# MECLabTUDA/Lifelong-nnUNet

Measured on AMD Instinct MI355X. Metric: 3D patches/sec (whole node) + mean Dice vs ref, 5-level 3D Generic_UNet training step, higher is better.
Workload: dtype f16 (fp32 accumulate, fp32 master weights); 1 GPU; BASELINE configs[1]: nnUNetTrainerSequential.run_iteration, 160x192x160 patches, batch 2/GPU, num_pool 5, base 32, 3 logits; global_batch=2, parallelism=dp1, distinct_resident_batches=2, deterministic_wgrad=False

## Files before the change

lifelong-nnunet_amd/csrc/igemm_conv.hip:

```cpp
#include "lnn_common.h"
#include "igemm_common.h"
#include "igemm_gen.h"
#include <cstdlib>

namespace {

typedef unsigned c1_uint4 __attribute__((ext_vector_type(4)));

template <bool STATS>
__global__ __launch_bounds__(256, 3) void conv_c1_fwd_kernel(const ConvParams p, int tiles_per_sample) {
    constexpr int TZ = 4, TY = 8, TX = 8, VT = TZ * TY * TX / 128, PZ = TZ + 2, PY = TY + 2, PX = TX + 2, P = PZ * PY * PX;
    constexpr int NL = (P + 255) / 256;
    __shared__ half_t xl[P];
    __shared__ float sred[STATS ? 4 * 2 * 32 : 1];
    const int tid = threadIdx.x, lane = tid & 63, wave = tid >> 6;
    const int n = blockIdx.y;
    const int m0 = blockIdx.z * 32;
    const long xbase_n = (long)n * p.Di * p.Hi * p.Wi;
    const int v = lane & 31, hk = lane >> 5;
    half8 a[2];
#pragma unroll
    for (int k16 = 0; k16 < 2; ++k16) a[k16] = *reinterpret_cast<const half8*>(p.wp + lnn_panel_off(0, m0 + v, k16 * 16 + hk * 8, 1, 32));
    int toff[2][8];
#pragma unroll
// ... 158 lines not shown
extern "C" int lnn_debug_set_gen_mode(int mode) {
    LNN_REQUIRE(mode >= -1 && mode <= 1, "lnn_debug_set_gen_mode: %d is not one of -1, 0, 1", mode);
    g_gen_mode = mode;
    return LNN_OK;
}
bool lnn_gen_prefers(int op, long voxels) {
    if (g_gen_mode >= 0) return g_gen_mode == 1;
    if (g_force_conv >= 0) return false;
    static int off = -1;
    if (off < 0) { const char* e = getenv("LNN_GEN"); off = (e && e[0] == '0') ? 1 : 0; }
    if (off) return false;
    switch (op) {
        case LNN_GEN_OP_CONV_S1: return voxels > 512 && voxels <= 4096;
        case LNN_GEN_OP_CONV_S2: return voxels <= 4096;
        case LNN_GEN_OP_CONVT_DGRAD: return voxels <= 20000;
        default: return false;
    }
}

namespace {
int check_act(const void* ptr, int ld, int C, const char* what) {
    LNN_REQUIRE(ptr != nullptr, "%s: null pointer", what);
    LNN_REQUIRE(lnn_aligned16(ptr), "%s: pointer not 16-byte aligned", what);
    LNN_REQUIRE(C > 0 && C % 8 == 0, "%s: channel count %d must be a positive multiple of 8", what, C);
    LNN_REQUIRE(ld >= C && ld % 8 == 0, "%s: ld %d must be >= C (%d) and a multiple of 8", what, ld, C);
    return LNN_OK;
}

}

// ... 328 lines not shown
```

lifelong-nnunet_amd/csrc/igemm_gen.h:

```cpp
#pragma once
#include "lnn_common.h"

typedef unsigned GenTap;
static inline GenTap gen_tap(int dz, int dy, int dx, int slot) {
    return (unsigned)(dz + 8) | ((unsigned)(dy + 8) << 8) | ((unsigned)(dx + 8) << 16) | ((unsigned)slot << 24);
}

struct GenParams {
    const half_t* x = nullptr;
    const half_t* wp = nullptr;
    const float* bias = nullptr;
    half_t* y = nullptr;
    float* scratch = nullptr;
    int ld_x = 0, ld_y = 0;
    int N = 0, Di = 0, Hi = 0, Wi = 0, Do = 0, Ho = 0, Wo = 0, Ld = 0, Lh = 0, Lw = 0;
    int soz = 1, soy = 1, sox = 1, siz = 1, siy = 1, six = 1;
    int C = 0, M = 0, Mpad = 0, KCpad = 0, wtaps = 0;
    int nclass = 0;
    int accumulate = 0, ksplit = 1;
    int vgroups = 0, mgroups = 0, nbpc = 0, xcd_order = 0;
    unsigned x_bytes = 0, wp_bytes = 0;
    GenTap taps[27] = {};
    unsigned cls_first[9] = {};
    unsigned cls_par[8] = {};
};

struct GenWParams {
    const half_t* p = nullptr;
    const half_t* q = nullptr;
    float* dwp = nullptr;
    float* parts = nullptr;
    long parts_elems = 0, part_stride = 0;
    int ld_p = 0, ld_q = 0;
    int N = 0, Ld = 0, Lh = 0, Lw = 0, Qd = 0, Qh = 0, Qw = 0;
    int siz = 1, siy = 1, six = 1;
    int M = 0, C = 0, Mpad = 0, Cpad = 0;
    int ntaps = 0, wtaps = 0, tgroups = 0, vparts = 1;
    unsigned p_bytes = 0, q_bytes = 0;
    GenTap taps[27] = {};
};

int lnn_gen_geometry(GenParams& p, int kind, const int k[3], const int st[3]);
int lnn_launch_gen(hipStream_t s, GenParams& p, float* ws, long ws_elems, const char* name);
int lnn_launch_gen_wgrad(hipStream_t s, GenWParams& p, const char* name);

int lnn_gen_conv3d_fwd(hipStream_t s, const void* x, int ld_x, const void* wp, const float* bias, void* y, int ld_y, int N, int Di,
                       int Hi, int Wi, int C, int K, const int k[3], const int st[3], float* ws, long ws_elems);
int lnn_gen_conv3d_dgrad(hipStream_t s, const void* dy, int ld_dy, const void* wp, void* dx, int ld_dx, int N, int Di, int Hi, int Wi,
                         int C, int K, const int k[3], const int st[3], int accumulate, float* ws, long ws_elems);
int lnn_gen_convT3d_fwd(hipStream_t s, const void* x, int ld_x, const void* wp, void* y, int ld_y, int N, int D, int H, int W, int C,
                        int K, const int st[3], float* ws, long ws_elems);
int lnn_gen_convT3d_dgrad(hipStream_t s, const void* dy, int ld_dy, const void* wp, void* dx, int ld_dx, int N, int D, int H, int W,
                          int C, int K, const int st[3], int accumulate, float* ws, long ws_elems);
int lnn_gen_conv3d_wgrad(hipStream_t s, const void* x, int ld_x, const void* dy, int ld_dy, float* dwp, int N, int Di, int Hi, int Wi,
                         int C, int K, const int k[3], const int st[3], float* parts, long parts_elems);
int lnn_gen_convT3d_wgrad(hipStream_t s, const void* x, int ld_x, const void* dy, int ld_dy, float* dwp, int N, int D, int H, int W,
                          int C, int K, const int st[3], float* parts, long parts_elems);
enum { LNN_GEN_OP_CONV_S1 = 0, LNN_GEN_OP_CONV_S2 = 1, LNN_GEN_OP_CONVT_FWD = 2, LNN_GEN_OP_CONVT_DGRAD = 3, LNN_GEN_OP_WGRAD = 4 };
bool lnn_gen_prefers(int op, long voxels);
```

lifelong-nnunet_amd/csrc/igemm_gen.hip:

```cpp
#include "igemm_common.h"
#include "igemm_gen.h"
#include <algorithm>

namespace {

typedef unsigned uint4v __attribute__((ext_vector_type(4)));
constexpr unsigned OOB = 0x80000000u;

__device__ __forceinline__ __amdgpu_buffer_rsrc_t gen_rsrc(const void* base, unsigned bytes) {
    return __builtin_amdgcn_make_buffer_rsrc(const_cast<void*>(base), 0, (int)bytes, 0x00020000);
}
__device__ __forceinline__ half8 gen_load16(__amdgpu_buffer_rsrc_t rs, unsigned off) {
    const uint4v r = __builtin_amdgcn_raw_buffer_load_b128(rs, (int)off, 0, 0);
    return __builtin_bit_cast(half8, r);
}

template <int RB, int VB, int D>
__global__ __launch_bounds__(256) void igemm_gen_kernel(const GenParams p) {
    const int lane = threadIdx.x & 63, wave = __builtin_amdgcn_readfirstlane(threadIdx.x >> 6);
    const int v = lane & 31, hk = lane >> 5;
    const int W = p.nclass * p.mgroups * p.ksplit;
    int w, vq;
    if (p.xcd_order) {
        const int xcd = blockIdx.x & 7, j = blockIdx.x >> 3;
// ... 121 lines not shown
                if (p.accumulate) {
                    const half4 old = *dst;
                    r0 += (float)old[0]; r1 += (float)old[1]; r2 += (float)old[2]; r3 += (float)old[3];
                }
                const half4 o = {(half_t)r0, (half_t)r1, (half_t)r2, (half_t)r3};
                *dst = o;
            }
        }
    }
}

typedef __attribute__((address_space(3))) void lds_void;
__device__ __forceinline__ void gen_dma16(__amdgpu_buffer_rsrc_t rs, char* lds_wave_base, unsigned voffset) {
    __builtin_amdgcn_raw_ptr_buffer_load_lds(rs, (lds_void*)lds_wave_base, 16, (int)voffset, 0, 0, 0);
}
__device__ __forceinline__ half4 gen_tr16(const char* addr) {
    fp16x4_t r = __builtin_amdgcn_ds_read_tr16_b64_v4f16((__attribute__((address_space(3))) fp16x4_t*)(addr));
    half4 o;
    __builtin_memcpy(&o, &r, 8);
    return o;
}
__device__ __forceinline__ half8 gen_tr_operand(const char* img, int p_addr) {
    const half4 lo = gen_tr16(img + p_addr), hi = gen_tr16(img + 256 + p_addr);
    half8 o;
#pragma unroll
    for (int i = 0; i < 4; ++i) { o[i] = lo[i]; o[4 + i] = hi[i]; }
    return o;
}
__device__ __forceinline__ int gen_div(int q, int d, float rd) {
    int r = (int)((float)q * rd);
    int rem = q - r * d;
    if (rem < 0) { --r; rem += d; }
    if (rem >= d) ++r;
    return r;
}

constexpr int GW_IMG = 1024;

template <int TPW>
__global__ __launch_bounds__(256) void igemm_gen_wgrad_kernel(const GenWParams p) {
    constexpr int WAVE_LDS = 2 * (1 + TPW) * GW_IMG;
    extern __shared__ __attribute__((aligned(16))) char smem[];
    const int lane = threadIdx.x & 63, wave = __builtin_amdgcn_readfirstlane(threadIdx.x >> 6);
    char* const lds = smem + wave * WAVE_LDS;
    const int panels = (p.Mpad >> 5) * (p.Cpad >> 5);
    const long units = (long)panels * p.tgroups * p.vparts;
    const long unit = (long)blockIdx.x * 4 + wave;
    if (unit >= units) return;
    const int vpart = (int)(unit % p.vparts);
    const int tg = (int)((unit / p.vparts) % p.tgroups);
    const int panel = (int)(unit / ((long)p.vparts * p.tgroups));
    const int m0 = (panel / (p.Cpad >> 5)) * 32, c0 = (panel % (p.Cpad >> 5)) * 32;
    const int t_begin = tg * TPW;
    const __amdgpu_buffer_rsrc_t rs_q = gen_rsrc(p.q, p.q_bytes);
    const __amdgpu_buffer_rsrc_t rs_p = gen_rsrc(p.p, p.p_bytes);

    const int dv = lane >> 2, dc = (lane & 3) * 8;
    const unsigned pcol = (m0 + dc < p.M) ? (unsigned)(m0 + dc) * 2u : OOB;
    const unsigned qcol = (c0 + dc < p.C) ? (unsigned)(c0 + dc) * 2u : OOB;
    const int hk = lane >> 5, cb = 16 * ((lane >> 4) & 1), sj = (lane & 15) >> 2, sq = lane & 3;
    const int p_addr = (8 * hk + sj) * 64 + (cb + 4 * sq) * 2;
    int tdz[TPW], tdy[TPW], tdx[TPW];
    unsigned tdead[TPW];
#pragma unroll
    for (int k = 0; k < TPW; ++k) {
        const bool has = t_begin + k < p.ntaps;
        const GenTap t = p.taps[has ? t_begin + k : 0];
        tdz[k] = (int)(t & 255) - 8; tdy[k] = (int)((t >> 8) & 255) - 8; tdx[k] = (int)((t >> 16) & 255) - 8;
        tdead[k] = has ? 0u : OOB;
    }

    floatx16 acc[TPW];
#pragma unroll
    for (int i = 0; i < TPW; ++i)
#pragma unroll
        for (int k = 0; k < 16; ++k) acc[i][k] = 0.f;

    const int total = p.N * p.Ld * p.Lh * p.Lw;
    const int groups = (total + 15) >> 4;
    const int g_begin = (int)((long)vpart * groups / p.vparts), g_end = (int)((long)(vpart + 1) * groups / p.vparts);
    const float rLw = 1.0f / (float)p.Lw, rLh = 1.0f / (float)p.Lh, rLd = 1.0f / (float)p.Ld;
    const unsigned prowb = (unsigned)p.ld_p * 2u, qrowb = (unsigned)p.ld_q * 2u;
#pragma unroll 1
    for (int gi = g_begin; gi < g_end; ++gi) {
        char* const buf = lds + (gi & 1) * (1 + TPW) * GW_IMG;
        const int q = gi * 16 + dv;
        const unsigned vdead = q < total ? 0u : OOB;
        const int qq = q < total ? q : 0;
        const int t1 = gen_div(qq, p.Lw, rLw), lx = qq - t1 * p.Lw;
        const int t2 = gen_div(t1, p.Lh, rLh), ly = t1 - t2 * p.Lh;
        const int n = gen_div(t2, p.Ld, rLd), lz = t2 - n * p.Ld;
        gen_dma16(rs_p, buf, (((unsigned)qq * prowb) | vdead | (pcol & OOB)) + (pcol & ~OOB));
        const int bz = lz * p.siz, by = ly * p.siy, bx = lx * p.six;
#pragma unroll
        for (int k = 0; k < TPW; ++k) {
            const int iz = bz + tdz[k], iy = by + tdy[k], ix = bx + tdx[k];
            const bool in = (unsigned)iz < (unsigned)p.Qd && (unsigned)iy < (unsigned)p.Qh && (unsigned)ix < (unsigned)p.Qw;
            const unsigned qrow = ((((unsigned)n * p.Qd + iz) * p.Qh + iy) * p.Qw + ix) * qrowb;
            gen_dma16(rs_q, buf + (1 + k) * GW_IMG, ((in ? qrow : OOB) | vdead | tdead[k] | (qcol & OOB)) + (qcol & ~OOB));
        }
        __builtin_amdgcn_s_waitcnt(0x0f70);
        __asm__ volatile("" ::: "memory");
        const half8 a = gen_tr_operand(buf, p_addr);
#pragma unroll
        for (int k = 0; k < TPW; ++k) {
            const half8 b = gen_tr_operand(buf + (1 + k) * GW_IMG, p_addr);
            acc[k] = __builtin_amdgcn_mfma_f32_32x32x16_f16(a, b, acc[k], 0, 0, 0);
        }
    }
    const int c = c0 + (lane & 31);
#pragma unroll
    for (int k = 0; k < TPW; ++k) {
        if (t_begin + k >= p.ntaps) continue;
        const int slot = (int)(p.taps[t_begin + k] >> 24);
#pragma unroll
        for (int i = 0; i < 16; ++i) {
            const int m = m0 + (i >> 2) * 8 + hk * 4 + (i & 3);
            const long idx = ((long)slot * p.Mpad + m) * p.Cpad + c;
            if (p.parts) p.parts[(long)vpart * p.part_stride + idx] = acc[k][i];
            else atomicAdd(p.dwp + idx, acc[k][i]);
        }
    }
}
// ... 90 lines not shown
    p.xcd_order = W % 8 == 0 ? 1 : 0;
    const unsigned grid = (unsigned)((long)W * p.nbpc);
    hipLaunchKernelGGL((igemm_gen_kernel<RB, VB, D>), dim3(grid), dim3(256), 0, s, p);
    LNN_CHECK_LAUNCH(name);
    if (ks > 1) {
        ConvParams c{};
        c.scratch = ws; c.ksplit = ks; c.Mpad = p.Mpad; c.M = p.M; c.bias = p.bias; c.y = p.y;
        c.ld_y = p.ld_y; c.accumulate = p.accumulate; c.N = p.N; c.Do = p.Do; c.Ho = p.Ho; c.Wo = p.Wo;
        return lnn_launch_splitk_finalize(s, c, name);
    }
    return LNN_OK;
}

template <int TPW>
static int gen_wgrad_launch_t(hipStream_t s, GenWParams& p, const char* name) {
    constexpr int WAVE_LDS = 2 * (1 + TPW) * GW_IMG;
    const long total = (long)p.N * p.Ld * p.Lh * p.Lw;
    p.tgroups = lnn_cdiv(p.ntaps, TPW);
    const long base = (long)(p.Mpad >> 5) * (p.Cpad >> 5) * p.tgroups;
    const int groups = (int)((total + 15) / 16);
    long vp = lnn_cdiv(8L * gen_num_cu(), base);
    if (vp > groups) vp = groups;
    if (vp < 1) vp = 1;
    const long slot_elems = (long)p.wtaps * p.Mpad * p.Cpad;
    if (p.parts) {
        while (vp > 1 && vp * slot_elems > p.parts_elems) --vp;
        LNN_REQUIRE(vp * slot_elems <= p.parts_elems, "%s: deterministic scratch too small (%ld floats needed, %ld given)", name,
                    vp * slot_elems, p.parts_elems);
        p.part_stride = slot_elems;
    }
    p.vparts = (int)vp;
    const long units = base * vp;
    auto kern = igemm_gen_wgrad_kernel<TPW>;
    static bool attr_set = false;
    if (!attr_set) {
        (void)hipFuncSetAttribute(reinterpret_cast<const void*>(kern), hipFuncAttributeMaxDynamicSharedMemorySize, 160 * 1024);
        attr_set = true;
    }
    hipLaunchKernelGGL(kern, dim3((unsigned)lnn_cdiv(units, 4)), dim3(256), (size_t)4 * WAVE_LDS, s, p);
    LNN_CHECK_LAUNCH(name);
    if (p.parts) {
        const long v4 = slot_elems / 4;
        const int blocks = (int)((v4 + 255) / 256 < 2048 ? (v4 + 255) / 256 : 2048);
        hipLaunchKernelGGL(gen_reduce_parts_kernel, dim3(blocks), dim3(256), 0, s, p.parts, (int)vp, slot_elems, p.dwp);
        LNN_CHECK_LAUNCH(name);
    }
    return LNN_OK;
}

int lnn_launch_gen_wgrad(hipStream_t s, GenWParams& p, const char* name) {
    const long total = (long)p.N * p.Ld * p.Lh * p.Lw;
    LNN_REQUIRE(total < (1L << 24), "%s: %ld loop voxels exceed the 2^24 the generic weight gradient indexes", name, total);
    const long pb = total * p.ld_p * 2, qb = (long)p.N * p.Qd * p.Qh * p.Qw * p.ld_q * 2;
    LNN_REQUIRE(pb < 0x7fffffffL && qb < 0x7fffffffL, "%s: tensor exceeds the 2 GB a buffer descriptor of the generic kernel covers", name);
    p.p_bytes = (unsigned)pb; p.q_bytes = (unsigned)qb;
    p.Mpad = lnn_round_up(p.M, 32); p.Cpad = lnn_round_up(p.C, 32);
    switch (p.ntaps) {
        case 27: return gen_wgrad_launch_t<7>(s, p, name);
        case 9: case 3: return gen_wgrad_launch_t<3>(s, p, name);
        case 8: case 4: return gen_wgrad_launch_t<4>(s, p, name);
        case 2: return gen_wgrad_launch_t<2>(s, p, name);
        case 1: return gen_wgrad_launch_t<1>(s, p, name);
    }
    lnn_set_error("%s: %d taps unsupported", name, p.ntaps);
    return LNN_ERR_BAD_ARG;
}

namespace {
int gen_check_act(const void* ptr, int ld, int C, const char* what) {
    LNN_REQUIRE(ptr != nullptr, "%s: null pointer", what);
    LNN_REQUIRE(lnn_aligned16(ptr), "%s: pointer not 16-byte aligned", what);
    LNN_REQUIRE(C > 0 && C % 8 == 0, "%s: channel count %d must be a positive multiple of 8", what, C);
    LNN_REQUIRE(ld >= C && ld % 8 == 0, "%s: ld %d must be >= C (%d) and a multiple of 8", what, ld, C);
    return LNN_OK;
// ... 64 lines not shown

int lnn_gen_convT3d_dgrad(hipStream_t s, const void* dy, int ld_dy, const void* wp, void* dx, int ld_dx, int N, int D, int H, int W,
                          int C, int K, const int st[3], int accumulate, float* ws, long ws_elems) {
    if (int e = gen_check_geom(st, st, true, "lnn_convT3d_dgrad_g")) return e;
    if (int e = gen_check_act(dy, ld_dy, K, "lnn_convT3d_dgrad_g(dy)")) return e;
    if (int e = gen_check_act(dx, ld_dx, C, "lnn_convT3d_dgrad_g(dx)")) return e;
    LNN_REQUIRE(wp != nullptr && lnn_aligned16(wp), "lnn_convT3d_dgrad_g: weight panel null/misaligned");
    GenParams p{};
    p.x = (const half_t*)dy; p.wp = (const half_t*)wp; p.y = (half_t*)dx; p.ld_x = ld_dy; p.ld_y = ld_dx;
    p.N = N; p.Di = D * st[0]; p.Hi = H * st[1]; p.Wi = W * st[2]; p.Do = D; p.Ho = H; p.Wo = W;
    p.Ld = D; p.Lh = H; p.Lw = W; p.C = K; p.M = C; p.accumulate = accumulate;
    lnn_gen_geometry(p, 3, st, st);
    return lnn_launch_gen(s, p, ws, ws_elems, "lnn_convT3d_dgrad_g");
}

int lnn_gen_conv3d_wgrad(hipStream_t s, const void* x, int ld_x, const void* dy, int ld_dy, float* dwp, int N, int Di, int Hi, int Wi,
                         int C, int K, const int k[3], const int st[3], float* parts, long parts_elems) {
    if (int e = gen_check_geom(k, st, false, "lnn_conv3d_wgrad_g")) return e;
    if (int e = gen_check_act(x, ld_x, C, "lnn_conv3d_wgrad_g(x)")) return e;
    if (int e = gen_check_act(dy, ld_dy, K, "lnn_conv3d_wgrad_g(dy)")) return e;
    LNN_REQUIRE(dwp != nullptr, "lnn_conv3d_wgrad_g: null panel");
    GenWParams p{};
    p.p = (const half_t*)dy; p.q = (const half_t*)x; p.dwp = dwp; p.ld_p = ld_dy; p.ld_q = ld_x; p.parts = parts; p.parts_elems = parts_elems;
    p.N = N; p.Qd = Di; p.Qh = Hi; p.Qw = Wi;
    p.Ld = (Di - 1) / st[0] + 1; p.Lh = (Hi - 1) / st[1] + 1; p.Lw = (Wi - 1) / st[2] + 1;
    p.siz = st[0]; p.siy = st[1]; p.six = st[2]; p.M = K; p.C = C;
    GenParams g{};
    p.ntaps = lnn_gen_geometry(g, 0, k, st);
    p.wtaps = g.wtaps;
    for (int t = 0; t < p.ntaps; ++t) p.taps[t] = g.taps[t];
    return lnn_launch_gen_wgrad(s, p, "lnn_conv3d_wgrad_g");
}

int lnn_gen_convT3d_wgrad(hipStream_t s, const void* x, int ld_x, const void* dy, int ld_dy, float* dwp, int N, int D, int H, int W,
                          int C, int K, const int st[3], float* parts, long parts_elems) {
    if (int e = gen_check_geom(st, st, true, "lnn_convT3d_wgrad_g")) return e;
    if (int e = gen_check_act(x, ld_x, C, "lnn_convT3d_wgrad_g(x)")) return e;
// ... 14 lines not shown
                                int Di, int Hi, int Wi, int C, int K, int kz, int ky, int kx, int sz, int sy, int sx, float* splitk_ws,
                                long splitk_elems) {
    const int k[3] = {kz, ky, kx}, st[3] = {sz, sy, sx};
    return lnn_gen_conv3d_fwd((hipStream_t)s, x, ld_x, wp, bias, y, ld_y, N, Di, Hi, Wi, C, K, k, st, splitk_ws, splitk_elems);
}
extern "C" int lnn_conv3d_dgrad_g(lnn_stream_t s, const void* dy, int ld_dy, const void* wp, void* dx, int ld_dx, int N, int Di, int Hi,
                                  int Wi, int C, int K, int kz, int ky, int kx, int sz, int sy, int sx, int accumulate, float* splitk_ws,
                                  long splitk_elems) {
    const int k[3] = {kz, ky, kx}, st[3] = {sz, sy, sx};
    return lnn_gen_conv3d_dgrad((hipStream_t)s, dy, ld_dy, wp, dx, ld_dx, N, Di, Hi, Wi, C, K, k, st, accumulate, splitk_ws, splitk_elems);
}
extern "C" int lnn_conv3d_wgrad_g(lnn_stream_t s, const void* x, int ld_x, const void* dy, int ld_dy, float* dwp, int N, int Di, int Hi,
                                  int Wi, int C, int K, int kz, int ky, int kx, int sz, int sy, int sx, float* parts, long parts_elems) {
    const int k[3] = {kz, ky, kx}, st[3] = {sz, sy, sx};
    LNN_REQUIRE(parts == nullptr || lnn_aligned16(parts), "lnn_conv3d_wgrad_g: scratch misaligned");
    return lnn_gen_conv3d_wgrad((hipStream_t)s, x, ld_x, dy, ld_dy, dwp, N, Di, Hi, Wi, C, K, k, st, parts, parts_elems);
}
extern "C" int lnn_convT3d_fwd_g(lnn_stream_t s, const void* x, int ld_x, const void* wp, void* y, int ld_y, int N, int D, int H, int W,
                                 int C, int K, int sz, int sy, int sx, float* splitk_ws, long splitk_elems) {
    const int st[3] = {sz, sy, sx};
    return lnn_gen_convT3d_fwd((hipStream_t)s, x, ld_x, wp, y, ld_y, N, D, H, W, C, K, st, splitk_ws, splitk_elems);
}
extern "C" int lnn_convT3d_dgrad_g(lnn_stream_t s, const void* dy, int ld_dy, const void* wp, void* dx, int ld_dx, int N, int D, int H,
                                   int W, int C, int K, int sz, int sy, int sx, int accumulate, float* splitk_ws, long splitk_elems) {
    const int st[3] = {sz, sy, sx};
    return lnn_gen_convT3d_dgrad((hipStream_t)s, dy, ld_dy, wp, dx, ld_dx, N, D, H, W, C, K, st, accumulate, splitk_ws, splitk_elems);
}
extern "C" int lnn_convT3d_wgrad_g(lnn_stream_t s, const void* x, int ld_x, const void* dy, int ld_dy, float* dwp, int N, int D, int H,
                                   int W, int C, int K, int sz, int sy, int sx, float* parts, long parts_elems) {
    const int st[3] = {sz, sy, sx};
    LNN_REQUIRE(parts == nullptr || lnn_aligned16(parts), "lnn_convT3d_wgrad_g: scratch misaligned");
// ... 3 lines not shown
```

lifelong-nnunet_amd/csrc/igemm_wgrad.hip:

```cpp
#include "lnn_common.h"
#include "igemm_gen.h"
#include <cstdlib>

namespace {

struct WTapTable {
    int ntaps;
    unsigned short pos_off[27];
    unsigned char slot[27];
};

struct WgradParams {
    const half_t* p;
    const half_t* q;
    const half_t* q2 = nullptr;
    int csplit = 0x7fffffff;
    float* dwp;
    int ld_p, ld_q;
    int N, Ld, Lh, Lw, Qd, Qh, Qw;
    int M, C, Mpad, Cpad;
    int tiles_z, tiles_y, tiles_x, tiles_total, tiles_per_block;
    int pad_lo;
    float* parts = nullptr;
    long parts_elems = 0, part_stride = 0;
// ... 955 lines not shown
        p.Cpad = 32;
        p.tiles_z = lnn_cdiv(p.Ld, TZ); p.tiles_y = lnn_cdiv(p.Lh, TY); p.tiles_x = lnn_cdiv(p.Lw, 8);
        p.tiles_total = N * p.tiles_z * p.tiles_y * p.tiles_x;
        int tpb = lnn_cdiv(p.tiles_total, 2048);
        if (tpb < 1) tpb = 1;
        p.tiles_per_block = tpb;
        dim3 grid((unsigned)lnn_cdiv(p.tiles_total, tpb), (unsigned)(p.Mpad / 32));
        const long slot_elems = (long)p.Mpad * 32;
        if (int e = wg_prepare_parts(p, grid.x, 4, slot_elems, "lnn_conv3d_wgrad(C=1)")) return e;
        if (p.gz) hipLaunchKernelGGL((wgrad_c1_kernel<TZ, TY, true>), grid, dim3(256), 0, s, p);
        else hipLaunchKernelGGL((wgrad_c1_kernel<TZ, TY, false>), grid, dim3(256), 0, s, p);
        LNN_CHECK_LAUNCH("lnn_conv3d_wgrad(C=1)");
        return wg_reduce_parts(s, p, grid.x, slot_elems, "lnn_conv3d_wgrad(C=1,reduce)");
    }
    if (int e = check_act_w(x, ld_x, x2 ? c_a : C, "lnn_conv3d_wgrad(x)")) return e;
    if (!x2 && lnn_gen_prefers(LNN_GEN_OP_WGRAD, (long)N * p.Ld * p.Lh * p.Lw)) {
        const int k3[3] = {3, 3, 3}, st3[3] = {stride, stride, stride};
        return lnn_gen_conv3d_wgrad(s, x, ld_x, dy, ld_dy, dwp, N, Di, Hi, Wi, C, K, k3, st3, parts, parts_elems);
    }
    p.taps.ntaps = 27;
    if (stride == 1) {
        constexpr int PY = 10, PX = 10;
        for (int t = 0; t < 27; ++t) {
            p.taps.pos_off[t] = (unsigned short)(((t / 9) * PY + (t / 3) % 3) * PX + t % 3);
            p.taps.slot[t] = (unsigned char)t;
        }
        LNN_REQUIRE(6L * p.Qh * p.Qw * p.ld_q * 2 < 0x7fffffffL && 4L * p.Lh * p.Lw * p.ld_p * 2 < 0x7fffffffL,
                    "lnn_conv3d_wgrad: a z-plane of %ld bytes is beyond the 2 GB window of the tile descriptors", (long)p.Qh * p.Qw * p.ld_q * 2);
        return launch_wgrad_s1_v5(s, p);
    }
    return launch_wgrad_s2<3>(s, p, "lnn_conv3d_wgrad(s2)");
}
}
// ... 70 lines not shown
```

lifelong-nnunet_amd/csrc/norm_act.hip:

```cpp
#include "igemm_common.h"

namespace {

constexpr int NT = 256;
typedef float float2v __attribute__((ext_vector_type(2)));
constexpr int MAX_BLOCKS = 1024;
constexpr int UNR = 4;

__device__ __forceinline__ half8 ld8(const half_t* p, int nt) {
    return nt ? __builtin_nontemporal_load(reinterpret_cast<const half8*>(p)) : *reinterpret_cast<const half8*>(p);
}
__device__ __forceinline__ void st8(half_t* p, const half8& v, int nt) {
    if (nt) __builtin_nontemporal_store(v, reinterpret_cast<half8*>(p));
    else *reinterpret_cast<half8*>(p) = v;
}
int in_nt_flag() {
    static int v = -1;
    if (v < 0) { const char* e = getenv("LNN_IN_NT"); v = (e && e[0] == '1') ? 1 : 0; }
    return v;
}

struct RowMap {
    int C8, VPB, c8, vl;
    bool active;
// ... 658 lines not shown
    }
    for (; v < end; v += step) {
        half8 pr;
        float d[KT];
        DlFetch<KT, QUAD> df;
        if (PRIOR) pr = *reinterpret_cast<const half8*>(dp + v * ld_dz);
        df.load(dln, V, v);
        df.get(d);
        *reinterpret_cast<half8*>(yp + v * C) = grad(*reinterpret_cast<const half8*>(yp + v * C), pr, d);
    }
}

constexpr int SNT = 512, SRL = SNT / 4;
constexpr int SMALL_V = SRL * 16;

__device__ __forceinline__ void small_block_sum16(float (&v)[16], double* red, double* dtot) {
    const int lane = threadIdx.x & 63, wid = threadIdx.x >> 6;
#pragma unroll
    for (int j = 0; j < 16; ++j) {
#pragma unroll
        for (int o = 32; o >= 4; o >>= 1) v[j] += __shfl_xor(v[j], o, 64);
    }
    __syncthreads();
    if (lane < 4) {
#pragma unroll
        for (int j = 0; j < 16; ++j) red[((lane * 16) + j) * (SNT / 64) + wid] = (double)v[j];
    }
    __syncthreads();
    if (threadIdx.x < 64) {
        double t = 0;
#pragma unroll
        for (int w = 0; w < SNT / 64; ++w) t += red[threadIdx.x * (SNT / 64) + w];
        dtot[threadIdx.x] = t;
    }
    __syncthreads();
}

constexpr int SU = 4;
__global__ __launch_bounds__(SNT) void in_small_fwd_kernel(const half_t* __restrict__ y, half_t* __restrict__ z, int ld_z, int V, int C,
                                                           float eps, const float* __restrict__ gamma, const float* __restrict__ beta,
                                                           float slope, float* __restrict__ mean, float* __restrict__ rstd) {
    __shared__ double red[64 * (SNT / 64)];
    __shared__ double dtot[64];
    __shared__ float bc[64];
    const int oc = threadIdx.x & 3, rl = threadIdx.x >> 2;
    const int n = blockIdx.y;
    const bool chan_ok = blockIdx.x * 32 + oc * 8 < C;
// ... 9 lines not shown
        for (int k = 0; k < SU; ++k) {
            const int r = r0 + k * SRL;
            x[k] = *reinterpret_cast<const half8*>(yn + (r < V ? r : V - 1) * C);
        }
#pragma unroll
        for (int k = 0; k < SU; ++k) {
            const bool live = r0 + k * SRL < V && chan_ok;
#pragma unroll
            for (int e = 0; e < 8; ++e) {
                const float f = live ? (float)x[k][e] : 0.f;
                part[e] += f;
                part[8 + e] += f * f;
            }
        }
    }
    small_block_sum16(part, red, dtot);
    if (threadIdx.x < 32) {
        const int o = threadIdx.x >> 3, e = threadIdx.x & 7, c = blockIdx.x * 32 + threadIdx.x;
        if (c < C) {
            const double m = dtot[o * 16 + e] / (double)V;
            double var = dtot[o * 16 + 8 + e] / (double)V - m * m;
            if (var < 0) var = 0;
            const float mf = (float)m, rf = (float)(1.0 / sqrt(var + (double)eps));
            mean[n * C + c] = mf; rstd[n * C + c] = rf;
            const float sc = gamma[c] * rf;
            bc[threadIdx.x] = sc;
            bc[32 + threadIdx.x] = beta[c] - mf * sc;
        }
    }
    __syncthreads();
    if (!chan_ok) return;
// ... 9 lines not shown
        }
#pragma unroll
        for (int k = 0; k < SU; ++k) {
            half8 o;
#pragma unroll
            for (int e = 0; e < 8; ++e) {
                const float t = (float)x[k][e] * sc[e] + sh[e];
                o[e] = (half_t)(t > 0.f ? t : t * slope);
            }
            const int r = r0 + k * SRL;
            if (r < V) *reinterpret_cast<half8*>(zn + r * ld_z) = o;
        }
    }
}

__global__ __launch_bounds__(SNT) void in_small_bwd_kernel(half_t* __restrict__ y, const half_t* __restrict__ dz, int ld_dz, int N, int V,
                                                           int C, const float* __restrict__ mean, const float* __restrict__ rstd,
                                                           const float* __restrict__ gamma, const float* __restrict__ beta, float slope,
                                                           double* __restrict__ ws, float* dgamma, float* dbeta, float unscale) {
    __shared__ double red[64 * (SNT / 64)];
    __shared__ double dtot[64];
    __shared__ float bc[64];
    const int oc = threadIdx.x & 3, rl = threadIdx.x >> 2;
    const bool chan_ok = blockIdx.x * 32 + oc * 8 < C;
    const int c0 = chan_ok ? blockIdx.x * 32 + oc * 8 : 0;
    float ga[8], be[8];
#pragma unroll
    for (int e = 0; e < 8; ++e) { ga[e] = gamma[c0 + e]; be[e] = beta[c0 + e]; }
    const float invV = 1.0f / (float)V;
    double gacc = 0;
    for (int n = 0; n < N; ++n) {
        float mu[8], rs[8];
#pragma unroll
        for (int e = 0; e < 8; ++e) { mu[e] = mean[n * C + c0 + e]; rs[e] = rstd[n * C + c0 + e]; }
        half_t* yn = y + (long)n * V * C + c0;
        const half_t* dn = dz + (long)n * V * ld_dz + c0;
        float part[16];
#pragma unroll
        for (int e = 0; e < 16; ++e) part[e] = 0.f;
        for (int r0 = rl; r0 < V; r0 += SU * SRL) {
            half8 xv[SU], gv[SU];
#pragma unroll
            for (int k = 0; k < SU; ++k) {
                const int r = r0 + k * SRL, rc = r < V ? r : V - 1;
                xv[k] = *reinterpret_cast<const half8*>(yn + rc * C);
                gv[k] = *reinterpret_cast<const half8*>(dn + rc * ld_dz);
            }
#pragma unroll
            for (int k = 0; k < SU; ++k) {
                const bool live = r0 + k * SRL < V && chan_ok;
#pragma unroll
                for (int e = 0; e < 8; ++e) {
                    const float h = ((float)xv[k][e] - mu[e]) * rs[e];
                    const float pre = ga[e] * h + be[e];
                    const float gg = live ? (float)gv[k][e] * (pre > 0.f ? 1.f : slope) : 0.f;
                    part[e] += gg;
                    part[8 + e] += gg * h;
                }
            }
        }
        small_block_sum16(part, red, dtot);
        if (threadIdx.x < 64) {
            const double t = dtot[threadIdx.x];
            const int o = threadIdx.x >> 4, j = threadIdx.x & 15, c = blockIdx.x * 32 + o * 8 + (j & 7);
            bc[threadIdx.x] = (float)(t * (double)invV);
            gacc += t;
            if (c < C) ws[((long)n * C + c) * 3 + (j >> 3)] = t;
        }
        __syncthreads();
        if (chan_ok) {
            float m1[8], m2[8];
#pragma unroll
            for (int e = 0; e < 8; ++e) { m1[e] = bc[oc * 16 + e]; m2[e] = bc[oc * 16 + 8 + e]; }
            for (int r0 = rl; r0 < V; r0 += SU * SRL) {
                half8 xv[SU], gv[SU];
#pragma unroll
                for (int k = 0; k < SU; ++k) {
                    const int r = r0 + k * SRL, rc = r < V ? r : V - 1;
                    xv[k] = *reinterpret_cast<const half8*>(yn + rc * C);
                    gv[k] = *reinterpret_cast<const half8*>(dn + rc * ld_dz);
                }
#pragma unroll
                for (int k = 0; k < SU; ++k) {
                    half8 o;
#pragma unroll
                    for (int e = 0; e < 8; ++e) {
                        const float h = ((float)xv[k][e] - mu[e]) * rs[e];
                        const float pre = ga[e] * h + be[e];
                        const float gg = (float)gv[k][e] * (pre > 0.f ? 1.f : slope);
                        o[e] = (half_t)(ga[e] * rs[e] * (gg - m1[e] - h * m2[e]));
                    }
                    const int r = r0 + k * SRL;
                    if (r < V) *reinterpret_cast<half8*>(yn + r * C) = o;
                }
            }
        }
    }
    if (threadIdx.x < 64) {
        const int o = threadIdx.x >> 4, j = threadIdx.x & 15, c = blockIdx.x * 32 + o * 8 + (j & 7);
        if (c < C) {
            if (j < 8) { if (dbeta) atomicAdd(dbeta + c, (float)(gacc * unscale)); }
            else if (dgamma) atomicAdd(dgamma + c, (float)(gacc * unscale));
        }
    }
}

bool small_enabled() {
    static int v = -1;
    if (v < 0) { const char* e = getenv("LNN_IN_SMALL"); v = (e && e[0] == '0') ? 0 : 1; }
    return v != 0;
}

int blocks_for(long V, int C) {
    const int vpb = NT / (C / 8);
// ... 18 lines not shown
                            const float* beta, float slope, float* mean, float* rstd) {
    if (int e = check_common(y, N, V, C, "lnn_conv3d_fwd_in_lrelu(norm)")) return e;
    LNN_REQUIRE(V <= SMALL_V, "lnn_conv3d_fwd_in_lrelu(norm): %ld voxels per sample exceed the single-launch limit %d", V, SMALL_V);
    LNN_REQUIRE(z != nullptr && lnn_aligned16(z) && ld_z >= C && ld_z % 8 == 0, "lnn_conv3d_fwd_in_lrelu(norm): bad z / ld_z");
    LNN_REQUIRE(mean && rstd && gamma && beta, "lnn_conv3d_fwd_in_lrelu(norm): null parameter");
    const dim3 grid(lnn_cdiv(C, 32), N);
    hipLaunchKernelGGL(in_small_fwd_kernel, grid, dim3(SNT), 0, s, (const half_t*)y, (half_t*)z, ld_z, (int)V, C, eps, gamma, beta, slope,
                       mean, rstd);
    LNN_CHECK_LAUNCH("lnn_conv3d_fwd_in_lrelu(norm)");
    return LNN_OK;
}

int lnn_launch_in_small_bwd(hipStream_t s, void* y, const void* dz, int ld_dz, int N, long V, int C, const float* mean, const float* rstd,
                            const float* gamma, const float* beta, float slope, double* ws, float* dgamma, float* dbeta, float unscale) {
    LNN_REQUIRE(V <= SMALL_V, "lnn_instnorm_lrelu_bwd(small): %ld voxels per sample exceed the single-launch limit %d", V, SMALL_V);
    hipLaunchKernelGGL(in_small_bwd_kernel, dim3(lnn_cdiv(C, 32)), dim3(SNT), 0, s, (half_t*)y, (const half_t*)dz, ld_dz, N, (int)V, C, mean,
                       rstd, gamma, beta, slope, ws, dgamma, dbeta, unscale);
    LNN_CHECK_LAUNCH("lnn_instnorm_lrelu_bwd(small)");
    return LNN_OK;
}

int lnn_launch_in_stats_finalize(hipStream_t s, const float* pws, int nslots, int N, int C, long V, float eps, float* mean, float* rstd) {
    hipLaunchKernelGGL(in_stats_finalize_kernel, dim3(lnn_cdiv(N * C, FEB)), dim3(256), 0, s, pws, nslots, N * C, V, eps, mean, rstd);
    LNN_CHECK_LAUNCH("lnn_instnorm_stats(finalize, fused partials)");
    return LNN_OK;
}

int lnn_launch_in_bwd_sums_raw(hipStream_t s, const float* pws, int nslots, int N, int C, const float* mean, const float* rstd,
                               double* ws, float* dgamma, float* dbeta, float unscale) {
    hipLaunchKernelGGL(in_lrelu_bwd_sums_kernel, dim3(lnn_cdiv(C, FEB)), dim3(256), 0, s, pws, nslots, N * C, C, ws, dgamma, dbeta,
                       unscale, mean, rstd);
// ... 165 lines not shown
```

Baseline: 105.0 patches/s.

## Deepen wgrad LDS ring, cost-model vparts, route concat wgrad, narrow small IN bwd

The generic wgrad kernel moves from double buffering to a deeper ring of up to four LDS buffers, waiting on only as many outstanding loads as needed, and it batches the transposed LDS reads through inline asm. Block-to-work mapping changes so each block covers one M panel. The volume split count now comes from a simple cost model that weighs group time against atomic traffic. The 27-tap case uses TPW=3 instead of 7, and the generic path now also handles concatenated (two-source) inputs through a channel split, which adds an env toggle. The small instance-norm backward kernel switches to 256 threads with 16 channels per block, giving more blocks for small C at the cost of more redundant per-block work.

```diff
diff --git a/lifelong-nnunet_amd/csrc/igemm_conv.hip b/lifelong-nnunet_amd/csrc/igemm_conv.hip
--- a/lifelong-nnunet_amd/csrc/igemm_conv.hip
+++ b/lifelong-nnunet_amd/csrc/igemm_conv.hip
@@ -196,6 +196,11 @@
         case LNN_GEN_OP_CONV_S1: return voxels > 512 && voxels <= 4096;
         case LNN_GEN_OP_CONV_S2: return voxels <= 4096;
         case LNN_GEN_OP_CONVT_DGRAD: return voxels <= 20000;
+        case LNN_GEN_OP_WGRAD: {
+            static int wg = -1;
+            if (wg < 0) { const char* e = getenv("LNN_GEN_WGRAD"); wg = (e && e[0] == '0') ? 0 : 1; }
+            return wg == 1 && voxels <= 4096;
+        }
         default: return false;
     }
 }
diff --git a/lifelong-nnunet_amd/csrc/igemm_gen.h b/lifelong-nnunet_amd/csrc/igemm_gen.h
--- a/lifelong-nnunet_amd/csrc/igemm_gen.h
+++ b/lifelong-nnunet_amd/csrc/igemm_gen.h
@@ -28,6 +28,8 @@
 struct GenWParams {
     const half_t* p = nullptr;
     const half_t* q = nullptr;
+    const half_t* q2 = nullptr;
+    int csplit = 0;
     float* dwp = nullptr;
     float* parts = nullptr;
     long parts_elems = 0, part_stride = 0;
@@ -52,8 +54,8 @@
                         int K, const int st[3], float* ws, long ws_elems);
 int lnn_gen_convT3d_dgrad(hipStream_t s, const void* dy, int ld_dy, const void* wp, void* dx, int ld_dx, int N, int D, int H, int W,
                           int C, int K, const int st[3], int accumulate, float* ws, long ws_elems);
-int lnn_gen_conv3d_wgrad(hipStream_t s, const void* x, int ld_x, const void* dy, int ld_dy, float* dwp, int N, int Di, int Hi, int Wi,
-                         int C, int K, const int k[3], const int st[3], float* parts, long parts_elems);
+int lnn_gen_conv3d_wgrad(hipStream_t s, const void* x, const void* x2, int c_a, int ld_x, const void* dy, int ld_dy, float* dwp, int N,
+                         int Di, int Hi, int Wi, int C, int K, const int k[3], const int st[3], float* parts, long parts_elems);
 int lnn_gen_convT3d_wgrad(hipStream_t s, const void* x, int ld_x, const void* dy, int ld_dy, float* dwp, int N, int D, int H, int W,
                           int C, int K, const int st[3], float* parts, long parts_elems);
 enum { LNN_GEN_OP_CONV_S1 = 0, LNN_GEN_OP_CONV_S2 = 1, LNN_GEN_OP_CONVT_FWD = 2, LNN_GEN_OP_CONVT_DGRAD = 3, LNN_GEN_OP_WGRAD = 4 };
diff --git a/lifelong-nnunet_amd/csrc/igemm_gen.hip b/lifelong-nnunet_amd/csrc/igemm_gen.hip
--- a/lifelong-nnunet_amd/csrc/igemm_gen.hip
+++ b/lifelong-nnunet_amd/csrc/igemm_gen.hip
@@ -159,18 +159,27 @@
 __device__ __forceinline__ void gen_dma16(__amdgpu_buffer_rsrc_t rs, char* lds_wave_base, unsigned voffset) {
     __builtin_amdgcn_raw_ptr_buffer_load_lds(rs, (lds_void*)lds_wave_base, 16, (int)voffset, 0, 0, 0);
 }
-__device__ __forceinline__ half4 gen_tr16(const char* addr) {
-    fp16x4_t r = __builtin_amdgcn_ds_read_tr16_b64_v4f16((__attribute__((address_space(3))) fp16x4_t*)(addr));
-    half4 o;
-    __builtin_memcpy(&o, &r, 8);
-    return o;
-}
-__device__ __forceinline__ half8 gen_tr_operand(const char* img, int p_addr) {
-    const half4 lo = gen_tr16(img + p_addr), hi = gen_tr16(img + 256 + p_addr);
+__device__ __forceinline__ half8 gen_join(half4 lo, half4 hi) {
     half8 o;
 #pragma unroll
     for (int i = 0; i < 4; ++i) { o[i] = lo[i]; o[4 + i] = hi[i]; }
     return o;
+}
+__device__ __forceinline__ void gen_tr1(unsigned addr, half8& x) {
+    half4 xl, xh;
+    __asm__ volatile("ds_read_b64_tr_b16 %0, %2\n\tds_read_b64_tr_b16 %1, %2 offset:256\n\ts_waitcnt lgkmcnt(0)"
+                     : "=&v"(xl), "=&v"(xh) : "v"(addr) : "memory");
+    x = gen_join(xl, xh);
+}
+__device__ __forceinline__ void gen_tr2(unsigned addr_x, unsigned addr_y, half8& x, half8& y) {
+    half4 xl, xh, yl, yh;
+    __asm__ volatile("ds_read_b64_tr_b16 %0, %4\n\tds_read_b64_tr_b16 %1, %4 offset:256\n\t"
+                     "ds_read_b64_tr_b16 %2, %5\n\tds_read_b64_tr_b16 %3, %5 offset:256\n\ts_waitcnt lgkmcnt(0)"
+                     : "=&v"(xl), "=&v"(xh), "=&v"(yl), "=&v"(yh) : "v"(addr_x), "v"(addr_y) : "memory");
+    x = gen_join(xl, xh); y = gen_join(yl, yh);
+}
+__device__ __forceinline__ unsigned gen_lds_addr(const char* ptr) {
+    return (unsigned)(__SIZE_TYPE__)(__attribute__((address_space(3))) const char*)ptr;
 }
 __device__ __forceinline__ int gen_div(int q, int d, float rd) {
     int r = (int)((float)q * rd);
@@ -181,30 +190,49 @@
 }
 
 constexpr int GW_IMG = 1024;
+constexpr double GW_GROUP_US = 0.2, GW_ATOMIC_BYTES_PER_US = 1.1e6;
+
+template <int N>
+__device__ __forceinline__ void gen_wait_vm() {
+    __builtin_amdgcn_s_waitcnt(0x0f70 | (N & 15) | ((N >> 4) << 14));
+}
+template <int A, int G>
+__device__ __forceinline__ void gen_wait_ahead(int ahead) {
+    if (ahead >= A) gen_wait_vm<A * G>();
+    else if constexpr (A > 0) gen_wait_ahead<A - 1, G>(ahead);
+}
+
+template <int TPW>
+struct GenWRing {
+    static constexpr int BUF = (1 + TPW) * GW_IMG;
+    static constexpr int NB = 16 * GW_IMG / BUF < 4 ? 16 * GW_IMG / BUF : 4;
+    static constexpr int WAVE_LDS = NB * BUF;
+};
 
 template <int TPW>
 __global__ __launch_bounds__(256) void igemm_gen_wgrad_kernel(const GenWParams p) {
-    constexpr int WAVE_LDS = 2 * (1 + TPW) * GW_IMG;
+    constexpr int BUF = GenWRing<TPW>::BUF, NB = GenWRing<TPW>::NB, WAVE_LDS = GenWRing<TPW>::WAVE_LDS;
     extern __shared__ __attribute__((aligned(16))) char smem[];
     const int lane = threadIdx.x & 63, wave = __builtin_amdgcn_readfirstlane(threadIdx.x >> 6);
     char* const lds = smem + wave * WAVE_LDS;
-    const int panels = (p.Mpad >> 5) * (p.Cpad >> 5);
-    const long units = (long)panels * p.tgroups * p.vparts;
-    const long unit = (long)blockIdx.x * 4 + wave;
-    if (unit >= units) return;
-    const int vpart = (int)(unit % p.vparts);
-    const int tg = (int)((unit / p.vparts) % p.tgroups);
-    const int panel = (int)(unit / ((long)p.vparts * p.tgroups));
-    const int m0 = (panel / (p.Cpad >> 5)) * 32, c0 = (panel % (p.Cpad >> 5)) * 32;
-    const int t_begin = tg * TPW;
-    const __amdgpu_buffer_rsrc_t rs_q = gen_rsrc(p.q, p.q_bytes);
+    const int ncp = p.Cpad >> 5;
+    const int upb = ncp * p.tgroups, bpm = (upb + 3) >> 2;
+    const int vpart = (int)(blockIdx.x % (unsigned)p.vparts);
+    const int rest = (int)(blockIdx.x / (unsigned)p.vparts);
+    const int unit = (rest % bpm) * 4 + wave;
+    if (unit >= upb) return;
+    const int m0 = (rest / bpm) * 32, c0 = (unit / p.tgroups) * 32;
+    const int t_begin = (unit % p.tgroups) * TPW;
+    const bool second = p.q2 != nullptr && c0 >= p.csplit;
+    const __amdgpu_buffer_rsrc_t rs_q = gen_rsrc(second ? p.q2 : p.q, p.q_bytes);
     const __amdgpu_buffer_rsrc_t rs_p = gen_rsrc(p.p, p.p_bytes);
 
     const int dv = lane >> 2, dc = (lane & 3) * 8;
     const unsigned pcol = (m0 + dc < p.M) ? (unsigned)(m0 + dc) * 2u : OOB;
-    const unsigned qcol = (c0 + dc < p.C) ? (unsigned)(c0 + dc) * 2u : OOB;
+    const unsigned qcol = (c0 + dc < p.C) ? (unsigned)(c0 - (second ? p.csplit : 0) + dc) * 2u : OOB;
     const int hk = lane >> 5, cb = 16 * ((lane >> 4) & 1), sj = (lane & 15) >> 2, sq = lane & 3;
     const int p_addr = (8 * hk + sj) * 64 + (cb + 4 * sq) * 2;
+    const unsigned lds_rd = gen_lds_addr(lds) + p_addr;
     int tdz[TPW], tdy[TPW], tdx[TPW];
     unsigned tdead[TPW];
 #pragma unroll
@@ -226,9 +254,7 @@
     const int g_begin = (int)((long)vpart * groups / p.vparts), g_end = (int)((long)(vpart + 1) * groups / p.vparts);
     const float rLw = 1.0f / (float)p.Lw, rLh = 1.0f / (float)p.Lh, rLd = 1.0f / (float)p.Ld;
     const unsigned prowb = (unsigned)p.ld_p * 2u, qrowb = (unsigned)p.ld_q * 2u;
-#pragma unroll 1
-    for (int gi = g_begin; gi < g_end; ++gi) {
-        char* const buf = lds + (gi & 1) * (1 + TPW) * GW_IMG;
+    auto issue = [&](int gi, char* buf) {
         const int q = gi * 16 + dv;
         const unsigned vdead = q < total ? 0u : OOB;
         const int qq = q < total ? q : 0;
@@ -244,14 +270,28 @@
             const unsigned qrow = ((((unsigned)n * p.Qd + iz) * p.Qh + iy) * p.Qw + ix) * qrowb;
             gen_dma16(rs_q, buf + (1 + k) * GW_IMG, ((in ? qrow : OOB) | vdead | tdead[k] | (qcol & OOB)) + (qcol & ~OOB));
         }
-        __builtin_amdgcn_s_waitcnt(0x0f70);
+    };
+#pragma unroll
+    for (int j = 0; j < NB - 1; ++j)
+        if (g_begin + j < g_end) issue(g_begin + j, lds + j * BUF);
+    int cur = 0;
+#pragma unroll 1
+    for (int gi = g_begin; gi < g_end; ++gi) {
+        const int last = cur == 0 ? NB - 1 : cur - 1;
+        __asm__ volatile("s_waitcnt lgkmcnt(0)" ::: "memory");
+        if (gi + NB - 1 < g_end) issue(gi + NB - 1, lds + last * BUF);
+        gen_wait_ahead<NB - 1, 1 + TPW>(g_end - 1 - gi);
         __asm__ volatile("" ::: "memory");
-        const half8 a = gen_tr_operand(buf, p_addr);
-#pragma unroll
-        for (int k = 0; k < TPW; ++k) {
-            const half8 b = gen_tr_operand(buf + (1 + k) * GW_IMG, p_addr);
-            acc[k] = __builtin_amdgcn_mfma_f32_32x32x16_f16(a, b, acc[k], 0, 0, 0);
+        const unsigned rd = lds_rd + cur * BUF;
+        half8 op[1 + TPW];
+#pragma unroll
+        for (int i = 0; i < 1 + TPW; i += 2) {
+            if (i + 1 < 1 + TPW) gen_tr2(rd + i * GW_IMG, rd + (i + 1) * GW_IMG, op[i], op[i + 1]);
+            else gen_tr1(rd + i * GW_IMG, op[i]);
+            if (i >= 1) acc[i - 1] = __builtin_amdgcn_mfma_f32_32x32x16_f16(op[0], op[i], acc[i - 1], 0, 0, 0);
+            if (i + 1 < 1 + TPW) acc[i] = __builtin_amdgcn_mfma_f32_32x32x16_f16(op[0], op[i + 1], acc[i], 0, 0, 0);
         }
+        cur = cur == NB - 1 ? 0 : cur + 1;
     }
     const int c = c0 + (lane & 31);
 #pragma unroll
@@ -372,15 +412,21 @@
 
 template <int TPW>
 static int gen_wgrad_launch_t(hipStream_t s, GenWParams& p, const char* name) {
-    constexpr int WAVE_LDS = 2 * (1 + TPW) * GW_IMG;
+    constexpr int WAVE_LDS = GenWRing<TPW>::WAVE_LDS;
     const long total = (long)p.N * p.Ld * p.Lh * p.Lw;
     p.tgroups = lnn_cdiv(p.ntaps, TPW);
-    const long base = (long)(p.Mpad >> 5) * (p.Cpad >> 5) * p.tgroups;
+    const long bpm = lnn_cdiv((long)(p.Cpad >> 5) * p.tgroups, 4);
+    const long base = (long)(p.Mpad >> 5) * bpm;
     const int groups = (int)((total + 15) / 16);
-    long vp = lnn_cdiv(8L * gen_num_cu(), base);
-    if (vp > groups) vp = groups;
-    if (vp < 1) vp = 1;
     const long slot_elems = (long)p.wtaps * p.Mpad * p.Cpad;
+    const long resident = 2L * gen_num_cu();
+    long vp = 1;
+    double best = 0;
+    for (long v = 1; v <= groups && v <= 64; ++v) {
+        const double t = (double)lnn_cdiv(base * v, resident) * (double)lnn_cdiv((long)groups, v) * GW_GROUP_US +
+                         (double)v * (double)slot_elems * 4.0 / GW_ATOMIC_BYTES_PER_US;
+        if (v == 1 || t < best) { best = t; vp = v; }
+    }
     if (p.parts) {
         while (vp > 1 && vp * slot_elems > p.parts_elems) --vp;
         LNN_REQUIRE(vp * slot_elems <= p.parts_elems, "%s: deterministic scratch too small (%ld floats needed, %ld given)", name,
@@ -388,14 +434,13 @@
         p.part_stride = slot_elems;
     }
     p.vparts = (int)vp;
-    const long units = base * vp;
     auto kern = igemm_gen_wgrad_kernel<TPW>;
     static bool attr_set = false;
     if (!attr_set) {
         (void)hipFuncSetAttribute(reinterpret_cast<const void*>(kern), hipFuncAttributeMaxDynamicSharedMemorySize, 160 * 1024);
         attr_set = true;
     }
-    hipLaunchKernelGGL(kern, dim3((unsigned)lnn_cdiv(units, 4)), dim3(256), (size_t)4 * WAVE_LDS, s, p);
+    hipLaunchKernelGGL(kern, dim3((unsigned)(base * vp)), dim3(256), (size_t)4 * WAVE_LDS, s, p);
     LNN_CHECK_LAUNCH(name);
     if (p.parts) {
         const long v4 = slot_elems / 4;
@@ -414,8 +459,7 @@
     p.p_bytes = (unsigned)pb; p.q_bytes = (unsigned)qb;
     p.Mpad = lnn_round_up(p.M, 32); p.Cpad = lnn_round_up(p.C, 32);
     switch (p.ntaps) {
-        case 27: return gen_wgrad_launch_t<7>(s, p, name);
-        case 9: case 3: return gen_wgrad_launch_t<3>(s, p, name);
+        case 27: case 9: case 3: return gen_wgrad_launch_t<3>(s, p, name);
         case 8: case 4: return gen_wgrad_launch_t<4>(s, p, name);
         case 2: return gen_wgrad_launch_t<2>(s, p, name);
         case 1: return gen_wgrad_launch_t<1>(s, p, name);
@@ -510,13 +554,18 @@
     return lnn_launch_gen(s, p, ws, ws_elems, "lnn_convT3d_dgrad_g");
 }
 
-int lnn_gen_conv3d_wgrad(hipStream_t s, const void* x, int ld_x, const void* dy, int ld_dy, float* dwp, int N, int Di, int Hi, int Wi,
-                         int C, int K, const int k[3], const int st[3], float* parts, long parts_elems) {
+int lnn_gen_conv3d_wgrad(hipStream_t s, const void* x, const void* x2, int c_a, int ld_x, const void* dy, int ld_dy, float* dwp, int N,
+                         int Di, int Hi, int Wi, int C, int K, const int k[3], const int st[3], float* parts, long parts_elems) {
     if (int e = gen_check_geom(k, st, false, "lnn_conv3d_wgrad_g")) return e;
-    if (int e = gen_check_act(x, ld_x, C, "lnn_conv3d_wgrad_g(x)")) return e;
+    if (int e = gen_check_act(x, ld_x, x2 ? c_a : C, "lnn_conv3d_wgrad_g(x)")) return e;
+    if (x2) {
+        LNN_REQUIRE(c_a % 32 == 0 && c_a < C, "lnn_conv3d_wgrad_g: split %d of %d channels must be a multiple of 32", c_a, C);
+        if (int e = gen_check_act(x2, ld_x, C - c_a, "lnn_conv3d_wgrad_g(x2)")) return e;
+    }
     if (int e = gen_check_act(dy, ld_dy, K, "lnn_conv3d_wgrad_g(dy)")) return e;
     LNN_REQUIRE(dwp != nullptr, "lnn_conv3d_wgrad_g: null panel");
     GenWParams p{};
+    p.q2 = (const half_t*)x2; p.csplit = x2 ? c_a : 0;
     p.p = (const half_t*)dy; p.q = (const half_t*)x; p.dwp = dwp; p.ld_p = ld_dy; p.ld_q = ld_x; p.parts = parts; p.parts_elems = parts_elems;
     p.N = N; p.Qd = Di; p.Qh = Hi; p.Qw = Wi;
     p.Ld = (Di - 1) / st[0] + 1; p.Lh = (Hi - 1) / st[1] + 1; p.Lw = (Wi - 1) / st[2] + 1;
@@ -561,7 +610,7 @@
                                   int Wi, int C, int K, int kz, int ky, int kx, int sz, int sy, int sx, float* parts, long parts_elems) {
     const int k[3] = {kz, ky, kx}, st[3] = {sz, sy, sx};
     LNN_REQUIRE(parts == nullptr || lnn_aligned16(parts), "lnn_conv3d_wgrad_g: scratch misaligned");
-    return lnn_gen_conv3d_wgrad((hipStream_t)s, x, ld_x, dy, ld_dy, dwp, N, Di, Hi, Wi, C, K, k, st, parts, parts_elems);
+    return lnn_gen_conv3d_wgrad((hipStream_t)s, x, nullptr, 0, ld_x, dy, ld_dy, dwp, N, Di, Hi, Wi, C, K, k, st, parts, parts_elems);
 }
 extern "C" int lnn_convT3d_fwd_g(lnn_stream_t s, const void* x, int ld_x, const void* wp, void* y, int ld_y, int N, int D, int H, int W,
                                  int C, int K, int sz, int sy, int sx, float* splitk_ws, long splitk_elems) {
diff --git a/lifelong-nnunet_amd/csrc/igemm_wgrad.hip b/lifelong-nnunet_amd/csrc/igemm_wgrad.hip
--- a/lifelong-nnunet_amd/csrc/igemm_wgrad.hip
+++ b/lifelong-nnunet_amd/csrc/igemm_wgrad.hip
@@ -993,9 +993,9 @@
         return wg_reduce_parts(s, p, grid.x, slot_elems, "lnn_conv3d_wgrad(C=1,reduce)");
     }
     if (int e = check_act_w(x, ld_x, x2 ? c_a : C, "lnn_conv3d_wgrad(x)")) return e;
-    if (!x2 && lnn_gen_prefers(LNN_GEN_OP_WGRAD, (long)N * p.Ld * p.Lh * p.Lw)) {
+    if (lnn_gen_prefers(LNN_GEN_OP_WGRAD, (long)N * p.Ld * p.Lh * p.Lw)) {
         const int k3[3] = {3, 3, 3}, st3[3] = {stride, stride, stride};
-        return lnn_gen_conv3d_wgrad(s, x, ld_x, dy, ld_dy, dwp, N, Di, Hi, Wi, C, K, k3, st3, parts, parts_elems);
+        return lnn_gen_conv3d_wgrad(s, x, x2, c_a, ld_x, dy, ld_dy, dwp, N, Di, Hi, Wi, C, K, k3, st3, parts, parts_elems);
     }
     p.taps.ntaps = 27;
     if (stride == 1) {
diff --git a/lifelong-nnunet_amd/csrc/norm_act.hip b/lifelong-nnunet_amd/csrc/norm_act.hip
--- a/lifelong-nnunet_amd/csrc/norm_act.hip
+++ b/lifelong-nnunet_amd/csrc/norm_act.hip
@@ -696,23 +696,24 @@
 constexpr int SNT = 512, SRL = SNT / 4;
 constexpr int SMALL_V = SRL * 16;
 
+template <int NT, int OCT>
 __device__ __forceinline__ void small_block_sum16(float (&v)[16], double* red, double* dtot) {
     const int lane = threadIdx.x & 63, wid = threadIdx.x >> 6;
 #pragma unroll
     for (int j = 0; j < 16; ++j) {
 #pragma unroll
-        for (int o = 32; o >= 4; o >>= 1) v[j] += __shfl_xor(v[j], o, 64);
+        for (int o = 32; o >= OCT; o >>= 1) v[j] += __shfl_xor(v[j], o, 64);
     }
     __syncthreads();
-    if (lane < 4) {
-#pragma unroll
-        for (int j = 0; j < 16; ++j) red[((lane * 16) + j) * (SNT / 64) + wid] = (double)v[j];
+    if (lane < OCT) {
+#pragma unroll
+        for (int j = 0; j < 16; ++j) red[((lane * 16) + j) * (NT / 64) + wid] = (double)v[j];
     }
     __syncthreads();
-    if (threadIdx.x < 64) {
+    if (threadIdx.x < OCT * 16) {
         double t = 0;
 #pragma unroll
-        for (int w = 0; w < SNT / 64; ++w) t += red[threadIdx.x * (SNT / 64) + w];
+        for (int w = 0; w < NT / 64; ++w) t += red[threadIdx.x * (NT / 64) + w];
         dtot[threadIdx.x] = t;
     }
     __syncthreads();
@@ -752,7 +753,7 @@
             }
         }
     }
-    small_block_sum16(part, red, dtot);
+    small_block_sum16<SNT, 4>(part, red, dtot);
     if (threadIdx.x < 32) {
         const int o = threadIdx.x >> 3, e = threadIdx.x & 7, c = blockIdx.x * 32 + threadIdx.x;
         if (c < C) {
@@ -792,16 +793,17 @@
     }
 }
 
-__global__ __launch_bounds__(SNT) void in_small_bwd_kernel(half_t* __restrict__ y, const half_t* __restrict__ dz, int ld_dz, int N, int V,
+constexpr int SBT = 256, SBO = 2, SBRL = SBT / SBO;
+__global__ __launch_bounds__(SBT) void in_small_bwd_kernel(half_t* __restrict__ y, const half_t* __restrict__ dz, int ld_dz, int N, int V,
                                                            int C, const float* __restrict__ mean, const float* __restrict__ rstd,
                                                            const float* __restrict__ gamma, const float* __restrict__ beta, float slope,
                                                            double* __restrict__ ws, float* dgamma, float* dbeta, float unscale) {
-    __shared__ double red[64 * (SNT / 64)];
-    __shared__ double dtot[64];
-    __shared__ float bc[64];
-    const int oc = threadIdx.x & 3, rl = threadIdx.x >> 2;
-    const bool chan_ok = blockIdx.x * 32 + oc * 8 < C;
-    const int c0 = chan_ok ? blockIdx.x * 32 + oc * 8 : 0;
+    __shared__ double red[SBO * 16 * (SBT / 64)];
+    __shared__ double dtot[SBO * 16];
+    __shared__ float bc[SBO * 16];
+    const int oc = threadIdx.x & (SBO - 1), rl = threadIdx.x / SBO;
+    const bool chan_ok = blockIdx.x * (SBO * 8) + oc * 8 < C;
+    const int c0 = chan_ok ? blockIdx.x * (SBO * 8) + oc * 8 : 0;
     float ga[8], be[8];
 #pragma unroll
     for (int e = 0; e < 8; ++e) { ga[e] = gamma[c0 + e]; be[e] = beta[c0 + e]; }
@@ -816,17 +818,17 @@
         float part[16];
 #pragma unroll
         for (int e = 0; e < 16; ++e) part[e] = 0.f;
-        for (int r0 = rl; r0 < V; r0 += SU * SRL) {
+        for (int r0 = rl; r0 < V; r0 += SU * SBRL) {
             half8 xv[SU], gv[SU];
 #pragma unroll
             for (int k = 0; k < SU; ++k) {
-                const int r = r0 + k * SRL, rc = r < V ? r : V - 1;
+                const int r = r0 + k * SBRL, rc = r < V ? r : V - 1;
                 xv[k] = *reinterpret_cast<const half8*>(yn + rc * C);
                 gv[k] = *reinterpret_cast<const half8*>(dn + rc * ld_dz);
             }
 #pragma unroll
             for (int k = 0; k < SU; ++k) {
-                const bool live = r0 + k * SRL < V && chan_ok;
+                const bool live = r0 + k * SBRL < V && chan_ok;
 #pragma unroll
                 for (int e = 0; e < 8; ++e) {
                     const float h = ((float)xv[k][e] - mu[e]) * rs[e];
@@ -837,10 +839,10 @@
                 }
             }
         }
-        small_block_sum16(part, red, dtot);
-        if (threadIdx.x < 64) {
+        small_block_sum16<SBT, SBO>(part, red, dtot);
+        if (threadIdx.x < SBO * 16) {
             const double t = dtot[threadIdx.x];
-            const int o = threadIdx.x >> 4, j = threadIdx.x & 15, c = blockIdx.x * 32 + o * 8 + (j & 7);
+            const int o = threadIdx.x >> 4, j = threadIdx.x & 15, c = blockIdx.x * (SBO * 8) + o * 8 + (j & 7);
             bc[threadIdx.x] = (float)(t * (double)invV);
             gacc += t;
             if (c < C) ws[((long)n * C + c) * 3 + (j >> 3)] = t;
@@ -850,11 +852,11 @@
             float m1[8], m2[8];
 #pragma unroll
             for (int e = 0; e < 8; ++e) { m1[e] = bc[oc * 16 + e]; m2[e] = bc[oc * 16 + 8 + e]; }
-            for (int r0 = rl; r0 < V; r0 += SU * SRL) {
+            for (int r0 = rl; r0 < V; r0 += SU * SBRL) {
                 half8 xv[SU], gv[SU];
 #pragma unroll
                 for (int k = 0; k < SU; ++k) {
-                    const int r = r0 + k * SRL, rc = r < V ? r : V - 1;
+                    const int r = r0 + k * SBRL, rc = r < V ? r : V - 1;
                     xv[k] = *reinterpret_cast<const half8*>(yn + rc * C);
                     gv[k] = *reinterpret_cast<const half8*>(dn + rc * ld_dz);
                 }
@@ -868,14 +870,14 @@
                         const float gg = (float)gv[k][e] * (pre > 0.f ? 1.f : slope);
                         o[e] = (half_t)(ga[e] * rs[e] * (gg - m1[e] - h * m2[e]));
                     }
-                    const int r = r0 + k * SRL;
+                    const int r = r0 + k * SBRL;
                     if (r < V) *reinterpret_cast<half8*>(yn + r * C) = o;
                 }
             }
         }
     }
-    if (threadIdx.x < 64) {
-        const int o = threadIdx.x >> 4, j = threadIdx.x & 15, c = blockIdx.x * 32 + o * 8 + (j & 7);
+    if (threadIdx.x < SBO * 16) {
+        const int o = threadIdx.x >> 4, j = threadIdx.x & 15, c = blockIdx.x * (SBO * 8) + o * 8 + (j & 7);
         if (c < C) {
             if (j < 8) { if (dbeta) atomicAdd(dbeta + c, (float)(gacc * unscale)); }
             else if (dgamma) atomicAdd(dgamma + c, (float)(gacc * unscale));
@@ -924,7 +926,7 @@
 int lnn_launch_in_small_bwd(hipStream_t s, void* y, const void* dz, int ld_dz, int N, long V, int C, const float* mean, const float* rstd,
                             const float* gamma, const float* beta, float slope, double* ws, float* dgamma, float* dbeta, float unscale) {
     LNN_REQUIRE(V <= SMALL_V, "lnn_instnorm_lrelu_bwd(small): %ld voxels per sample exceed the single-launch limit %d", V, SMALL_V);
-    hipLaunchKernelGGL(in_small_bwd_kernel, dim3(lnn_cdiv(C, 32)), dim3(SNT), 0, s, (half_t*)y, (const half_t*)dz, ld_dz, N, (int)V, C, mean,
+    hipLaunchKernelGGL(in_small_bwd_kernel, dim3(lnn_cdiv(C, SBO * 8)), dim3(SBT), 0, s, (half_t*)y, (const half_t*)dz, ld_dz, N, (int)V, C, mean,
                        rstd, gamma, beta, slope, ws, dgamma, dbeta, unscale);
     LNN_CHECK_LAUNCH("lnn_instnorm_lrelu_bwd(small)");
     return LNN_OK;
```

Result: no change. 105.9 patches/s, median of 6 (+0.8%).
